# tuffy/libdvd-audio

Measured on AMD Instinct MI355X. Metric: decoded PCM Msamples/s (bit-exact) on 6ch/96k/24b MLP, higher is better.
Workload: dtype int32 (int64 accumulate)

## Files before the change

libdvd-audio_amd/csrc/mlp_decode.h:

```cpp
#pragma once
#include <hip/hip_runtime.h>
#if defined(__HIP_DEVICE_COMPILE__) && !defined(__gfx950__)
#error "mlp_decode.h is written for gfx950 (MI355X): hand-placed s_waitcnt encodings and gfx950 inline asm"
#endif
#include <stdint.h>
#include <type_traits>
#include "mlp_bounds.h"
#include "mlp_index.h"
#include "mlp_tables.h"

namespace mlp {

constexpr int DEC_THREADS = 128;
constexpr int DEC_WAVES = DEC_THREADS / 64;
constexpr int MAXCH = 8;
constexpr int MAXMAT = 6;
constexpr int RING_PLANES = 8;
constexpr int RING_DWORDS = RING_PLANES * 4;
constexpr int CHUNK_DWORDS = 16;
constexpr int OUT_ROWS = 4;
constexpr uint32_t YIELD_LONELY = 48;
#ifndef DVDA_HDR_GATE_TURNS
#define DVDA_HDR_GATE_TURNS 32
#endif
// ... 638 lines not shown
    Reader rx;
    rx.gsrc = rd.gsrc;
    rx.ring = &s_ring[wv][0][0][lane];
    rx.max_chunk = rd.max_chunk;
    rx.pos = 0;
    rx.fillpos = 0;
    rx.lo_valid = 0;
    SubPark P0;
    P0.flags = 0xFF;
    P0.block_size = 8;
    P0.min_ch = P0.max_ch = P0.max_mat_ch = P0.noise_shift = P0.seed = P0.matrix_len = P0.bypass_mask = P0.outch_pack = 0;
    P0.oshift_pack = P0.qss_pack = P0.nslots = P0.iir_any = P0.ss_end_bit = P0.rows_left = P0.blocks_in_frame = 0;
    P0.have_restart = false;
    P0.seg_iir = false;
    P0.gl = segi * 2u;
    P0.seg_lane = P0.gl;
    P0.chk = (DUO && active) ? DVDA_AT(a.seg_check, (size_t)segi * 2u, 2ull * a.caps.max_seg, BT_CHECK) : 0xFFFFFFFFu;
    P0.brec = P0.brec_end = P0.brec_base = nullptr;
    if (DUO && PARSE && active) {
        const uint4 pl = DVDA_AT(a.plan, segi, a.caps.max_seg + 1u, BT_PLAN);
        P0.brec = a.brec + brec_offset(pl.x, pl.y, 0u, seg_R);
        P0.brec_base = P0.brec;
        P0.brec_end = P0.brec + brec_capacity(seg_R);
        if (!DVDA_RANGE_OK(brec_offset(pl.x, pl.y, 0u, seg_R), brec_capacity(seg_R), a.caps.brec, BT_BREC)) {
            status |= ST_CAPACITY;
            active = false;
        }
    }

    uint64_t sp[NS][4];
    auto st_get = [&](int k, int j) -> int32_t {
        return (j & 1) ? (int32_t)(uint32_t)(sp[k][j >> 1] >> 32) : (int32_t)(uint32_t)sp[k][j >> 1];
    };
    auto st_set = [&](int k, int j, int32_t v) {
        if (j & 1)
            sp[k][j >> 1] = (sp[k][j >> 1] & 0xFFFFFFFFull) | ((uint64_t)(uint32_t)v << 32);
        else
            sp[k][j >> 1] = (sp[k][j >> 1] & 0xFFFFFFFF00000000ull) | (uint32_t)v;
    };
    constexpr bool CFU = !PARSE && !GENERAL && !DUO;
    constexpr int CFW = CFU ? 8 : 4;
    int32_t cf[NS][CFW];
    uint32_t pk[NS];
    int32_t sho[NS];
    uint32_t mreg[2][4];
    uint32_t mnoise[2] = {0, 0};
    constexpr bool MU = ILV && !PAIRED && !GENERAL && !PARSE && !DUO;
    int32_t mu[2][MU ? 8 : 1];
#pragma unroll
    for (int m = 0; m < 2; m++)
#pragma unroll
        for (int j = 0; j < (MU ? 8 : 1); j++)
            mu[m][j] = 0;
#pragma unroll
    for (int k = 0; k < NS; k++) {
#pragma unroll
        for (int j = 0; j < 4; j++)
            sp[k][j] = 0;
#pragma unroll
        for (int j = 0; j < CFW; j++)
            cf[k][j] = 0;
        pk[k] = hot_word(0u, 24u, 0u, 0u);
        s_cold[wv][k][lane] = (uint16_t)cold_word(0u, 0u, 0u, 0u);
        sho[k] = -(1 << 23);
    }
#pragma unroll
    for (int m = 0; m < 2; m++)
#pragma unroll
        for (int j = 0; j < 4; j++)
            mreg[m][j] = 0;
    if (GENERAL && resume_from_init) {
#pragma unroll
        for (int k = 0; k < NS; k++)
#pragma unroll
            for (int j = 0; j < 8; j++)
                st_set(k, j, a.init_fir[((size_t)sr.stream * 2 + sub) * 48 + k * 8 + j]);
    }
    uint32_t flags = 0xFF;
    uint32_t block_size = 8;
    uint32_t min_ch = 0, max_ch = 0, max_mat_ch = 0, noise_shift = 0, seed = 0;
    uint32_t matrix_len = 0, bypass_mask = 0, outch_pack = 0;
    uint32_t oshift_pack = 0, qss_pack = 0;
    uint32_t qss_A = 0, mmc_A = 0;
    uint32_t gate_turn = 0;
    auto no_restart_yet = [&]() -> uint32_t {
        if (GENERAL)
            return ST_ENVELOPE;
        const uint32_t first = a.streams[a.seg[segi].stream].first_seg;
        return segi != first ? ST_SEQ : ST_ENVELOPE;
    };
    constexpr bool HDR_GATE = !PAIRED && !GENERAL;
    const uint32_t gl_r = gl;
    uint32_t nslots = 0;
    bool have_restart = false;
    uint32_t iir_any = 0;
    bool seg_iir = false;

    uint64_t cur = sr.off;
    uint32_t ss_end_bit = 0;
    uint32_t rows_left = 0;
    bool in_frame = false;
    uint32_t frame_rows = 0;
    uint32_t blocks_in_frame = 0;
    uint32_t frames_done = 0;
    uint64_t row = row0;
    uint32_t rows_written = 0;
// ... 16 lines not shown
        sw(max_ch, P0.max_ch);
        sw(max_mat_ch, P0.max_mat_ch);
        sw(noise_shift, P0.noise_shift);
        sw(seed, P0.seed);
        sw(matrix_len, P0.matrix_len);
        sw(bypass_mask, P0.bypass_mask);
        sw(outch_pack, P0.outch_pack);
        sw(oshift_pack, P0.oshift_pack);
        sw(qss_pack, P0.qss_pack);
        sw(nslots, P0.nslots);
        sw(iir_any, P0.iir_any);
        sw(ss_end_bit, P0.ss_end_bit);
        sw(rows_left, P0.rows_left);
        sw(blocks_in_frame, P0.blocks_in_frame);
        sw(chk, P0.chk);
        sw(gl, P0.gl);
        sw(seg_lane, P0.seg_lane);
        swb(have_restart, P0.have_restart);
        swb(seg_iir, P0.seg_iir);
        swp(brec, P0.brec);
        swp(brec_end, P0.brec_end);
        swp(brec_base, P0.brec_base);
        dsub ^= 1u;
    };

    auto rematrix = [&](int32_t(&ch)[MAXCH], uint32_t bypass_bits) {
        const uint32_t shifted = (seed >> 7) & 0xFFFFu;
        const int32_t n0 = (int32_t)((uint32_t)(int32_t)(int8_t)(seed >> 15) << noise_shift);
        const int32_t n1 = (int32_t)((uint32_t)(int32_t)(int8_t)shifted << noise_shift);
        seed = (seed << 16) ^ shifted ^ (shifted << 5);
        auto one_matrix = [&](const uint32_t(&mc)[4], uint32_t nz, uint32_t m, bool on) {
            int64_t acc = (int64_t)n0 * (int64_t)lo16(nz) + (int64_t)n1 * (int64_t)hi16(nz);
#pragma unroll
            for (int c = 0; c < 6; c++)
                acc += (int64_t)ch[c] * (int64_t)((c & 1) ? hi16(mc[c >> 1]) : lo16(mc[c >> 1]));
            const uint32_t oc = nib(outch_pack, m);
            const int32_t nv = (int32_t)((uint32_t)mask_q((int32_t)(acc >> 14), nib(qss_A, oc)) +
                                         ((bypass_bits >> m) & 1u));
            uint32_t oce = on ? oc : 0xFFu;
            asm volatile("" : "+v"(oce));
            uint64_t hit[6];
#pragma unroll
            for (int c = 0; c < 6; c++) {
                hit[c] = __builtin_amdgcn_ballot_w64((uint32_t)c == oce);
                asm volatile("" : "+s"(hit[c]));
            }
#pragma unroll
            for (int c = 0; c < 6; c++) {
                int32_t keep = ch[c];
                asm("v_cndmask_b32_e64 %0, %0, %1, %2" : "+v"(keep) : "v"(nv), "s"(hit[c]));
                ch[c] = keep;
            }
        };
        auto one_matrix_u = [&](const int32_t(&c8)[MU ? 8 : 1], uint32_t m, bool on) {
            int64_t acc = (int64_t)n0 * (int64_t)c8[MU ? 6 : 0] + (int64_t)n1 * (int64_t)c8[MU ? 7 : 0];
#pragma unroll
            for (int c = 0; c < 6; c++)
                acc += (int64_t)ch[c] * (int64_t)c8[MU ? c : 0];
            const uint32_t oc = nib(outch_pack, m);
            const int32_t nv = (int32_t)((uint32_t)mask_q((int32_t)(acc >> 14), nib(qss_A, oc)) +
                                         ((bypass_bits >> m) & 1u));
            uint32_t oce = on ? oc : 0xFFu;
            asm volatile("" : "+v"(oce));
            uint64_t hit[6];
#pragma unroll
            for (int c = 0; c < 6; c++) {
                hit[c] = __builtin_amdgcn_ballot_w64((uint32_t)c == oce);
                asm volatile("" : "+s"(hit[c]));
            }
#pragma unroll
            for (int c = 0; c < 6; c++) {
                int32_t keep = ch[c];
                asm("v_cndmask_b32_e64 %0, %0, %1, %2" : "+v"(keep) : "v"(nv), "s"(hit[c]));
                ch[c] = keep;
            }
        };
        if constexpr (MU) {
            if (__any(matrix_len > 0))
                one_matrix_u(mu[0], 0, matrix_len > 0);
            if (__any(matrix_len > 1))
                one_matrix_u(mu[1], 1, matrix_len > 1);
        } else {
        if (__any(matrix_len > 0))
            one_matrix(mreg[0], mnoise[0], 0, matrix_len > 0);
        if (__any(matrix_len > 1))
            one_matrix(mreg[1], mnoise[1], 1, matrix_len > 1);
        }
        if (GENERAL && __builtin_expect(__any(matrix_len > 2), 0)) {
            for (uint32_t m = 2; m < matrix_len; m++) {
                DVDA_COV(9);
                uint32_t mc[4];
#pragma unroll
                for (int j = 0; j < 4; j++)
                    mc[j] = a.mat_ws[(size_t)(m * 5 + j) * a.total_lanes + gl_r];
                one_matrix(mc, a.mat_ws[(size_t)(m * 5 + 4) * a.total_lanes + gl_r], m, true);
            }
        }
        if (__any(oshift_pack != 0)) {
#pragma unroll
            for (int c = 0; c < MAXCH; c++)
                if ((uint32_t)c <= mmc_A)
                    ch[c] = (int32_t)((uint32_t)ch[c] << nib(oshift_pack, c));
        }
    };

#if defined(DVDA_EXP_STAMP)
    unsigned long long stamp_acc[8] = {0, 0, 0, 0, 0, 0, 0, 0};
    unsigned long long stamp_t = clock64();
    unsigned long long hstamp_acc[6] = {0, 0, 0, 0, 0, 0};
    unsigned long long hfills = 0, hcount = 0;
    unsigned long long hstamp_t = 0;
#endif
    for (;;) {
        DVDA_STAMP(5);
        bool hdr_parsed = false;
        bool hdr_now = active && (rows_left == 0 || (DUO && P0.rows_left == 0));
        if (HDR_GATE && __builtin_expect(__any(hdr_now), 0)) {
            const uint64_t m_need = __ballot(hdr_now), m_act = __ballot(active);
            const bool go = m_need == m_act || (uint32_t)__popcll(m_need) >= HDR_GATE_LANES ||
                            (gate_turn & (HDR_GATE_TURNS - 1u)) == 0u;
            hdr_now = hdr_now && go;
        }
        gate_turn++;
        if (__builtin_expect(hdr_now, 0)) {
#if defined(DVDA_EXP_STAMP)
            hstamp_t = clock64();
            rd.fill_cyc = rd.fill_n = 0;
            if constexpr (DUO)
                rx.fill_cyc = rx.fill_n = 0;
#endif
            while (active && !in_frame) {
                if (frames_done == sr.nframes) {
                    if (GENERAL && a.fir_ws) {
#pragma unroll
                        for (int k = 0; k < NS; k++)
#pragma unroll
                            for (int j = 0; j < 8; j++)
                                a.fir_ws[(size_t)(k * 8 + j) * a.total_lanes + seg_lane] = st_get(k, j);
                    }
                    if (GENERAL || PARSE)
                        a.seg_meta[seg_lane] = min_ch | (max_ch << 4) | (1u << 8) | (seg_iir ? 1u << 9 : 0u);
                    if (PARSE && brec) {
#pragma unroll
                        for (int kk = 0; kk < 6; kk++)
                            brec[BREC_SLOT * kk] = 0xFFFFFFFFu;
                    }
                    if constexpr (DUO && PARSE) {
                        a.seg_meta[P0.seg_lane] = P0.min_ch | (P0.max_ch << 4) | (1u << 8) | (P0.seg_iir ? 1u << 9 : 0u);
                        if (P0.brec) {
#pragma unroll
                            for (int kk = 0; kk < 6; kk++)
                                P0.brec[BREC_SLOT * kk] = 0xFFFFFFFFu;
                        }
                    }
                    bool go_on = false;
                    if (GENERAL) {
                        atomicOr(&a.seg_status[segi], status | ((status & ~ST_INFO) ? 0u : ST_GENERAL));
                        if (is_last_sub)
                            a.seg_rows[segi] = rows_written;
                        uint32_t nxt = segi + 1;
                        while (nxt < n_seg && a.seg[nxt].stream == sr.stream && (a.seg[nxt].flags & SEG_DEAD))
                            nxt++;
                        if (!(status & ~ST_INFO) && nxt < n_seg) {
                            const SegRec nr = DVDA_AT(a.seg, nxt, a.caps.max_seg, BT_SEG);
                            const uint32_t nst = DVDA_AT(a.seg_status, nxt, a.caps.max_seg, BT_STATUS);
                            if (nr.stream == sr.stream && !(nr.flags & ST_FATAL_INDEX) && nr.nframes &&
                                !(nst & ~ST_INFO)) {
                                go_on = true;
                                atomicAnd(&a.seg_status[nxt], ST_DEFERRED | ST_FATAL_INDEX | ST_TRUNCATED | ST_SYNC_CHANGE);
                                seg_lane += (nxt - segi) * 2u;
                                segi = nxt;
                                sr = nr;
                                cur = nr.off;
                                frames_done = 0;
                                drops_seen = 0;
                                rows_written = 0;
// ... 144 lines not shown
                        if (restart) {
                            flags = rd.read_resident(1) ? rd.read_resident(8) : 0xFFu;
                        } else if ((flags & 0x80u) && rd.read_resident(1)) {
                            flags = rd.read_resident(8);
                        }
                        if ((flags & 0x01u) && rd.read_resident(1)) {
                            block_size = rd.read_resident(9);
                            if (block_size < 8)
                                ok = false;
                        } else if (restart) {
                            block_size = 8;
                        }
                        if (ok && (flags & 0x02u) && rd.read_resident(1)) {
                            if (blocks_in_frame)
                                matrix_class_change = true;
                            matrix_len = rd.read_resident(4);
                            if (matrix_len > MAXMAT) {
                                ok = false;
                                err = ST_ENVELOPE;
                                matrix_len = 0;
                            }
                            bypass_mask = 0;
                            outch_pack = 0;
                            for (uint32_t m = 0; m < matrix_len && ok; m++) {
                                rd.ensure(HDR_MATRIX);
                                const uint32_t oc = rd.read_resident(4);
                                const uint32_t frac = rd.read_resident(4);
                                if (oc > max_mat_ch || frac > 14) {
                                    ok = false;
                                    break;
                                }
                                outch_pack |= oc << (4 * m);
                                bypass_mask |= rd.read_resident(1) << m;
                                uint32_t pair = 0, noise = 0;
                                for (uint32_t c = 0; c < 10; c++) {
                                    int32_t v = 0;
                                    if (c < max_mat_ch + 3 && rd.read_resident(1))
                                        v = (int32_t)((uint32_t)rd.read_signed_resident(frac + 2) << (14 - frac));
                                    if (c == max_mat_ch + 1)
                                        noise |= (uint32_t)v & 0xFFFFu;
                                    if (c == max_mat_ch + 2)
                                        noise |= (uint32_t)v << 16;
                                    const int32_t vc = c <= max_mat_ch ? v : 0;
                                    if (c & 1) {
                                        const uint32_t word = pair | ((uint32_t)vc << 16);
                                        if (c < 8) {
                                            a.mat_ws[(size_t)(m * 5 + (c >> 1)) * a.total_lanes + gl] = word;
#pragma unroll
                                            for (int mm = 0; mm < 2; mm++)
#pragma unroll
                                                for (int jj = 0; jj < 4; jj++)
                                                    if ((uint32_t)mm == m && (uint32_t)jj == (c >> 1) && mat_mine) {
                                                        mreg[mm][jj] = word;
                                                        if constexpr (MU) {
                                                            if (jj < 3) {
                                                                mu[mm][MU ? 2 * jj : 0] = lo16(word);
                                                                mu[mm][MU ? 2 * jj + 1 : 0] = hi16(word);
                                                            }
                                                        }
                                                    }
                                        }
                                    } else {
                                        pair = (uint32_t)vc & 0xFFFFu;
                                    }
                                }
                                a.mat_ws[(size_t)(m * 5 + 4) * a.total_lanes + gl] = noise;
                                if (m == 0 && mat_mine)
                                    mnoise[0] = noise;
                                if (m == 1 && mat_mine)
                                    mnoise[1] = noise;
                                if constexpr (MU) {
#pragma unroll
                                    for (int mm = 0; mm < 2; mm++)
                                        if ((uint32_t)mm == m && mat_mine) {
                                            mu[mm][MU ? 6 : 0] = lo16(noise);
                                            mu[mm][MU ? 7 : 0] = hi16(noise);
                                        }
                                }
                            }
                        } else if (restart) {
                            matrix_len = 0;
                            bypass_mask = 0;
                        }
                        if (ok && (flags & 0x04u) && rd.read_resident(1)) {
                            if (blocks_in_frame)
                                matrix_class_change = true;
                            for (uint32_t c = 0; c <= max_mat_ch; c++) {
                                const int32_t v = rd.read_signed_resident(4);
                                if (v < 0) {
                                    ok = false;
                                    err = ST_ENVELOPE;
                                }
                                oshift_pack = (oshift_pack & ~(0xFu << (4 * c))) | (((uint32_t)v & 0xFu) << (4 * c));
                            }
                        } else if (restart) {
                            oshift_pack = 0;
                        }
                        bool qss_changed = false;
                        if (ok && (flags & 0x08u) && rd.read_resident(1)) {
                            if (blocks_in_frame)
                                matrix_class_change = true;
                            for (uint32_t c = 0; c <= max_ch; c++)
                                qss_pack = (qss_pack & ~(0xFu << (4 * c))) | (rd.read_resident(4) << (4 * c));
                            qss_changed = true;
                        } else if (restart) {
                            qss_pack = 0;
                            qss_changed = true;
                        }
                        DVDA_HSTAMP(2);
                        for (uint32_t k = 0; k < nslots && ok; k++) {
                            rd.ensure(HDR_FIR);
                            const uint32_t c = min_ch + k;
                            const uint32_t kr = DUO ? c : k;
                            uint32_t pk_old = 0;
                            int32_t sho_old = 0;
                            uint32_t cf_old[4] = {0, 0, 0, 0};
#pragma unroll
                            for (int kk = 0; kk < NS; kk++)
                                if ((uint32_t)kk == kr) {
                                    pk_old = pk[kk];
                                    sho_old = sho[kk];
                                    if (PARSE) {
#pragma unroll
                                        for (int j = 0; j < 4; j++)
                                            cf_old[j] = !CFU ? (uint32_t)cf[kk][CFU ? 0 : j]
                                                             : (((uint32_t)cf[kk][CFU ? 2 * j : 0] & 0xFFFFu) |
                                                                ((uint32_t)cf[kk][CFU ? 2 * j + 1 : 0] << 16));
                                    }
                                }
                            uint32_t codebook = hot_cb(pk_old);
// ... 156 lines not shown
                                        const bool with_iir = new_iir && iir_order != 0;
                                        if (brec + 2 * BREC_STRIDE + (with_iir ? BREC_IIR_WORDS : 0) > brec_end) {
                                            seq_needed = true;
                                        } else {
                                            uint32_t *w = brec + BREC_SLOT * k;
                                            w[2] = shift | (q << 4) | (fir_order << 8) | (iir_order << 12) |
                                                   (new_iir ? 1u << 16 : 0u);
#pragma unroll
                                            for (int j = 0; j < 4; j++)
                                                w[3 + j] = new_fir ? ncf[j] : cf_old[j];
                                            w[7] = 0;
                                            chg_mask |= 1u << k;
                                            if (with_iir) {
                                                const int32_t *ws = a.iir_ws + (size_t)(k * 16) * a.total_lanes + gl;
                                                brec_end -= BREC_IIR_WORDS;
                                                uint32_t *x = brec_end;
                                                for (uint32_t j = 0; j < 4; j++)
                                                    x[j] = ((uint32_t)ws[(size_t)(2 * j) * a.total_lanes] & 0xFFFFu) |
                                                           ((uint32_t)ws[(size_t)(2 * j + 1) * a.total_lanes] << 16);
                                                for (uint32_t j = 0; j < 8; j++)
                                                    x[4 + j] = (uint32_t)ws[(size_t)(8 + j) * a.total_lanes];
                                                w[7] = (uint32_t)(x - brec_base);
                                            }
                                        }
                                    }
                                }
                            }
                        }
                    }
                }
                DVDA_HSTAMP(3);
                if (!have_restart && ok) {
                    ok = false;
                    err = no_restart_yet();
                }
                hdr_parsed = true;
                if (PARSE && iir_any)
                    seg_iir = true;
                if (PARSE && ok && chg_mask) {
#pragma unroll
                    for (int kk = 0; kk < 6; kk++) {
                        brec[BREC_SLOT * kk] = rows_done;
                        brec[BREC_SLOT * kk + 1] = (chg_mask >> kk) & 1u;
                    }
                    brec += BREC_STRIDE;
                }
                if (PARSE && ok && (seq_needed || (hdr_restart && blocks_in_frame))) {
                    status |= ST_SEQ;
                    active = false;
                }
                if (mat_mine) {
                    qss_A = qss_pack;
                    mmc_A = max_mat_ch;
                }
                const uint32_t cold_ml = matrix_len;
                if (matrix_class_change)
                    status |= ST_MIDFRAME;
                if (!ok) {
                    status |= err;
                    active = false;
                } else if (PARSE && !active) {
                } else if (!GENERAL && !PARSE && (iir_any != 0 || cold_ml > 2)) {
                    status |= ST_COLD;
                    active = false;
                } else if (!GENERAL && !PARSE && (status & ST_CHAINED)) {
                    active = false;
                    if (!(DUO && probe))
                        atomicAdd(&s_nchained[wv], 1u);
                    if (sr.prev != 0xFFFFFFFFu)
                        __hip_atomic_store(&DVDA_AT(a.yield_req, sr.prev, a.caps.max_seg, BT_YIELD), 1u, __ATOMIC_RELAXED, __HIP_MEMORY_SCOPE_AGENT);
                } else {
                    rows_left = block_size;
                    blocks_in_frame++;
                    if (!GENERAL && !PARSE && frames_done < 2 &&
                        __hip_atomic_load(&s_nchained[wv], __ATOMIC_RELAXED, __HIP_MEMORY_SCOPE_WORKGROUP) >= YIELD_LONELY) {
                        status |= ST_YIELD;
                        active = false;
                    }
                }
            }
                if constexpr (DUO) {
                    if (pass == 0u && me)
                        swap_sub();
                    if (!PARSE && pass == 0u && me && !active && first0 && !(status & ~ST_INFO)) {
                        probe = true;
                        active = true;
                    }
                    if (pass == 1u && probe)
                        active = false;
                }
            }
            if constexpr (DUO) {
                if (active && have_restart && P0.have_restart && (P0.min_ch != 0u || min_ch != P0.max_ch + 1u)) {
                    status |= PARSE ? ST_SEQ : ST_COLD;
                    active = false;
                }
            }
        }
        if (hdr_now) {
            DVDA_HSTAMP(4);
#if defined(DVDA_EXP_STAMP)
            hstamp_acc[5] += rd.fill_cyc + (DUO ? rx.fill_cyc : 0ull);
            hfills += rd.fill_n + (DUO ? rx.fill_n : 0ull);
            hcount++;
#endif
        }
        if (!__any(active))
            break;
        DVDA_STAMP(0);

        if (active) {
            if constexpr (DUO) {
                while (__builtin_expect(__any(rd.ahead() < 8 || rx.ahead() < 8), 0)) {
                    DVDA_COV(14);
                    uint4 q[1];
                    const int32_t n0 = rx.template fill_issue<1>(q);
                    rx.template fill_commit<1>(q, n0);
                    const int32_t n1 = rd.template fill_issue<1>(q);
                    rd.template fill_commit<1>(q, n1);
                }
            } else {
            if (rd.ahead() < 12)
                DVDA_COV(14);
            rd.ensure(12);
            }
        }
        DVDA_STAMP(7);
        constexpr int32_t FILL_TURN = 16;
        const bool pf = !WAVE_FILL && active && rd.room();
        const bool pfx = DUO && active && rx.room();
        int32_t fn = 0;
        uint4 p0, p1, p2, p3;
        asm volatile("" : "=v"(p0.x), "=v"(p0.y), "=v"(p0.z), "=v"(p0.w), "=v"(p1.x), "=v"(p1.y), "=v"(p1.z), "=v"(p1.w),
                          "=v"(p2.x), "=v"(p2.y), "=v"(p2.z), "=v"(p2.w), "=v"(p3.x), "=v"(p3.y), "=v"(p3.z), "=v"(p3.w));
        bool flush = false;
        const uint32_t frames_before = frames_done;
        uint64_t flush_row = 0;
        if constexpr (DUO) {
            if (pfx)
                p0 = rx.gsrc[rx.fill_src() >> 2];
            if (pf)
                p1 = rd.gsrc[rd.fill_src() >> 2];
        } else if constexpr (WAVE_FILL) {
            if (__any(active && rd.ahead() <= FILL_TURN)) {
                const int32_t r = (RD - rd.ahead()) >> 2;
                fn = active ? (r < 4 ? r : 4) : 0;
                const uint32_t end = rd.max_chunk + (uint32_t)CHUNK_DWORDS;
                const uint32_t last = end - 4u * (uint32_t)fn;
                const uint4 *src = rd.gsrc + ((rd.fillpos < last ? rd.fillpos : last) >> 2);
                if (fn > 0)
                    p0 = src[0];
                if (fn > 1)
                    p1 = src[1];
                if (fn > 2)
                    p2 = src[2];
                if (fn > 3)
                    p3 = src[3];
            }
        } else {
        if (pf) {
            const uint32_t c = rd.fillpos < rd.max_chunk ? rd.fillpos : rd.max_chunk;
            const uint4 *src = rd.gsrc + (c >> 2);
            p0 = src[0];
            p1 = src[1];
            p2 = src[2];
            p3 = src[3];
        }
        }
// ... 74 lines not shown
                    (void)wave_iir;
                } else {
                auto tap = [&](int j) -> int32_t {
                    if constexpr (CFU)
                        return cf[k][CFU ? j : 0];
                    else
                        return (j & 1) ? hi16((uint32_t)cf[k][CFU ? 0 : j >> 1]) : lo16((uint32_t)cf[k][CFU ? 0 : j >> 1]);
                };
                int64_t acc0 = (int64_t)tap(0) * (int64_t)st_get(k, 0);
                int64_t acc1 = (int64_t)tap(1) * (int64_t)st_get(k, 1);
                acc0 += (int64_t)tap(2) * (int64_t)st_get(k, 2);
                acc1 += (int64_t)tap(3) * (int64_t)st_get(k, 3);
                acc0 += (int64_t)tap(4) * (int64_t)st_get(k, 4);
                acc1 += (int64_t)tap(5) * (int64_t)st_get(k, 5);
                acc0 += (int64_t)tap(6) * (int64_t)st_get(k, 6);
                acc1 += (int64_t)tap(7) * (int64_t)st_get(k, 7);
                int64_t acc = acc0 + acc1;
                bool iir_on = false;
                if (__builtin_expect(wave_iir, 0)) {
                    iir_on = in && ((iir_any >> k) & 1u);
                    if (iir_on)
                        DVDA_COV(11);
                    if (iir_on)
                        acc += iir_mac(a.iir_ws + (size_t)(k * 16) * a.total_lanes + gl, a.total_lanes);
                }
                value = (int32_t)(((uint32_t)(acc >> ((hw >> 10) & 63u)) + resq) << q5);
                {
                    uint32_t vhi;
                    asm("" : "=v"(vhi));
                    const uint64_t vpair = (uint64_t)(uint32_t)value | ((uint64_t)vhi << 32);
                    asm("v_pk_mov_b32 %0, %1, %0 op_sel:[1,0]" : "+v"(sp[k][3]) : "v"(sp[k][2]));
                    asm("v_pk_mov_b32 %0, %1, %0 op_sel:[1,0]" : "+v"(sp[k][2]) : "v"(sp[k][1]));
                    asm("v_pk_mov_b32 %0, %1, %0 op_sel:[1,0]" : "+v"(sp[k][1]) : "v"(sp[k][0]));
                    asm("v_pk_mov_b32 %0, %1, %0 op_sel:[0,0]" : "+v"(sp[k][0]) : "v"(vpair));
                }
                if (__builtin_expect(wave_iir, 0)) {
                    if (iir_on) {
                        const int32_t ssum = (int32_t)(acc >> (((hw >> 10) & 63u) - hot_q(hw)));
                        iir_push(a.iir_ws + (size_t)(k * 16) * a.total_lanes + gl, a.total_lanes,
                                 (int32_t)((uint32_t)value - (uint32_t)ssum));
                    }
                }
                }
                val[k] = value;
                }
            }
            rd.pos = cpos;
            if (__builtin_expect((msb_or & 0x80u) != 0, 0)) {
                status |= ST_HUFFMAN;
                active = false;
            }
            DVDA_STAMP(2);
        };
        auto row_tail = [&](int32_t (&ch)[MAXCH]) {
            if (owner) {
                if (GENERAL) {
                    if (frame_rows >= (uint32_t)FB_ROWS) {
                        status |= ST_ENVELOPE;
                        active = false;
                    } else {
                        int32_t *fr = fbuf + (size_t)frame_rows * (MAXCH + 1);
#pragma unroll
                        for (int c = 0; c < MAXCH; c++)
                            fr[c] = ch[c];
                        fr[MAXCH] = (int32_t)bypass_bits;
                    }
                } else {
                    if constexpr (PARSE) {
#pragma unroll
                        for (int j = 0; j < OUT_ROWS - 1; j++) {
                            pq_s[j] = pq_s[j + 1];
                        }
                        pq_s[OUT_ROWS - 1] = (int32_t)((seed & 0x7FFFFFu) | (bypass_bits << 23));
                        const uint32_t shifted = (seed >> 7) & 0xFFFFu;
                        seed = (seed << 16) ^ shifted ^ (shifted << 5);
                    } else {
                        rematrix(ch, bypass_bits);
                    }
                    const uint32_t ph = rows_done & (OUT_ROWS - 1);
                    int32_t(*T)[OUT_ROWS][GENERAL ? 1 : 64] =
                        s_out[GENERAL ? 0 : wv];
                    if (ILV && ilv_direct) {
                        int32_t *Td = &T[0][0][GENERAL ? 0 : lane] + ph * (6 * 64);
#pragma unroll
                        for (int c = 0; c < 6; c++)
                            Td[c * 64] = ch[c];
                    } else {
#pragma unroll
                        for (int c = 0; c < TP; c++)
                            T[c][ph][GENERAL ? 0 : lane] = ch[c];
                    }
                    if (__builtin_expect(room == 0, 0)) {
                        if (row >= out_stride && row < row_limit) {
                            status |= ST_OVERFLOW;
                            active = false;
                        }
                    } else {
                        rows_written++;
                        if (ph == OUT_ROWS - 1) {
                            flush = true;
                            flush_row = row - (OUT_ROWS - 1);
                        }
                    }
                }
            }
            row++;
            rows_done++;
            if (GENERAL) {
                if (row > row_limit) {
                    status |= ST_TIMING;
                    active = false;
                }
            } else if (__builtin_expect(room == 0, 0)) {
                if (row > row_limit) {
                    status |= ST_TIMING;
                    active = false;
                }
            } else {
                room--;
            }
            frame_rows++;
            rows_left--;
            if constexpr (DUO) {
                P0.rows_left--;
                if (__builtin_expect(active && (rows_left == 0 || P0.rows_left == 0), 0)) {
                    bool last0 = false, last1 = false;
                    if (P0.rows_left == 0) {
                        last0 = rx.read(1) != 0;
                        if (rx.past(P0.ss_end_bit)) {
                            status |= ST_EOF;
                            active = false;
                        }
                        if (active && last0 && (P0.chk >> 2) == frames_done) {
                            status |= (P0.chk & 1u) ? ST_PARITY : ST_CRC;
                            active = false;
                        }
                    }
                    if (active && rows_left == 0) {
                        last1 = rd.read(1) != 0;
                        if (rd.past(ss_end_bit)) {
                            status |= ST_EOF;
                            active = false;
                        }
                        if (active && last1 && (chk >> 2) == frames_done) {
                            status |= (chk & 1u) ? ST_PARITY : ST_CRC;
                            active = false;
                        }
                    }
                    if (active && (last0 || last1) && (!(last0 && last1) || frame_rows != rpa)) {
                        status |= ST_TIMING;
                        active = false;
                    }
                    if (last0 && last1) {
                        if (PARSE && active) {
                            uint32_t *F = frec + (size_t)au_idx * FREC_WORDS;
                            if (!DVDA_RANGE_OK((size_t)(F - a.frec), FREC_WORDS, a.caps.frec, BT_FREC))
                                F = a.frec;
                            F[0] = noise_shift | (matrix_len << 8) | (max_mat_ch << 16);
                            F[1] = outch_pack;
                            F[2] = qss_pack;
                            F[3] = oshift_pack;
#pragma unroll
                            for (int m = 0; m < 2; m++) {
#pragma unroll
                                for (int j = 0; j < 4; j++)
                                    F[4 + m * 5 + j] = mreg[m][j];
                                F[4 + m * 5 + 4] = mnoise[m];
                            }
                            for (uint32_t m = 2; m < matrix_len; m++)
                                for (uint32_t j = 0; j < 5; j++)
                                    F[4 + m * 5 + j] = a.mat_ws[(size_t)(m * 5 + j) * a.total_lanes + gl];
                        }
// ... 55 lines not shown
                                    uint8_t *wb = reinterpret_cast<uint8_t *>(a.pcm + out_base) + orow * nch_out * nb;
                                    for (uint32_t c = 0; c < nch_out && c < 6u; c++) {
                                        int32_t v = 0;
#pragma unroll
                                        for (int cc = 0; cc < 6; cc++)
                                            if ((uint32_t)cc == c)
                                                v = ch[cc];
                                        const uint32_t u = wav_signed(v, a.wav_bits);
                                        for (uint32_t b = 0; b < nb; b++)
                                            wb[nib(wavepk, c) * nb + b] = (uint8_t)(u >> (8 * b));
                                    }
                                } else {
#pragma unroll
                                for (int c = 0; c < 6; c++)
                                    if ((uint32_t)c < nch_out)
                                        a.pcm[out_base + (a.interleaved ? orow * nch_out + nib(wavepk, c)
                                                                        : (uint64_t)nib(wavepk, c) * out_stride + orow)] = ch[c];
                                }
                            }
                            rows_written++;
                        }
                    }
                    in_frame = false;
                    frames_done++;
                } else if (rd.past(ss_end_bit)) {
                    status |= ST_EOF;
                    active = false;
                }
            }
        };
        int32_t ch[MAXCH];
        const bool in_row = active && (!HDR_GATE || (rows_left != 0 && (!DUO || P0.rows_left != 0)));
        if (in_row) {
            row_head_any();
            if (PAIRED) {
                const int slot0 = lane & ~1;
                int32_t(*X)[XCH ? 64 : 1] = s_xch[XCH ? wv : 0];
#pragma unroll
                for (int k = 0; k < NS; k++)
                    if ((uint32_t)k < nslots && min_ch + k < MAXCH)
                        X[min_ch + k][XCH ? slot0 : 0] = val[k];
                __builtin_amdgcn_fence(__ATOMIC_RELEASE, "wavefront");
                __builtin_amdgcn_wave_barrier();
                __builtin_amdgcn_fence(__ATOMIC_ACQUIRE, "wavefront");
#pragma unroll
                for (int c = 0; c < MAXCH; c++)
                    ch[c] = X[c][XCH ? slot0 : 0];
            } else {
#pragma unroll
                for (int c = 0; c < MAXCH; c++)
                    ch[c] = c < NS ? val[c < NS ? c : 0] : 0;
            }
            row_tail(ch);
        }
        if constexpr (GENERAL) {
            const int ended = frames_done != frames_before ? 1 : 0;
            const int other = __shfl_xor(ended, 1, 64);
            if (S == 2u && active && ended != other) {
                status |= ST_ENVELOPE;
                active = false;
            }
        }
        DVDA_STAMP(3);

#if defined(DVDA_EXP_STAMP)
        {
            asm volatile("s_waitcnt vmcnt(0)" ::: "memory");
            DVDA_STAMP(6);
        }
#endif
        __builtin_amdgcn_s_waitcnt(0x0F70);
        if constexpr (DUO) {
            if (pfx) {
                ring_store4<RD>(rx.slot(rx.fillpos), p0, (rx.fillpos & (RD - 1)) == 0);
                rx.filled();
            }
            if (pf) {
                ring_store4<RD>(rd.slot(rd.fillpos), p1, (rd.fillpos & (RD - 1)) == 0);
                rd.filled();
            }
        } else if constexpr (WAVE_FILL) {
            if (__any(fn > 0)) {
                const uint32_t f = rd.fillpos;
                if (fn > 0) {
                    ring_store4<RD>(rd.slot(f), p0, (f & (RD - 1)) == 0);
                    if (fn > 1) {
                        ring_store4<RD>(rd.slot(f + 4u), p1, ((f + 4u) & (RD - 1)) == 0);
                        if (fn > 2) {
                            ring_store4<RD>(rd.slot(f + 8u), p2, ((f + 8u) & (RD - 1)) == 0);
                            if (fn > 3)
                                ring_store4<RD>(rd.slot(f + 12u), p3, ((f + 12u) & (RD - 1)) == 0);
                        }
                    }
                    rd.fillpos = f + 4u * (uint32_t)fn;
                    if (rd.fillpos - rd.lo_valid > (uint32_t)RD)
                        rd.lo_valid = rd.fillpos - RD;
                }
            }
        } else {
        if (pf) {
            ring_store16(rd.slot(rd.fillpos), p0, p1, p2, p3, (rd.fillpos & (RING_DWORDS - 1)) == 0);
            rd.filled();
        }
        }
        bool coop_out = false;
        if constexpr (ILV && !GENERAL && !PARSE) {
            if (!WAVO && ilv_direct && a.wav_bits == 0u && a.coop_min_seg && n_seg >= a.coop_min_seg)
                coop_out = __ballot(flush) == ~0ull;
        }
        if (coop_out) {
            const uint64_t doff = out_base + flush_row * 6u;
            const bool off32 = !__any((doff >> 32) != 0);
            const uint32_t d_lo = (uint32_t)doff, d_hi = (uint32_t)(doff >> 32);
            const int32_t *const T0 = &s_out[GENERAL ? 0 : wv][0][0][0];
            const uint32_t l6 = ((uint32_t)lane * 43691u) >> 18;
            const uint32_t pc = (uint32_t)lane - l6 * 6u;
            const int32_t *const Tl6 = T0 + pc * (4 * 64) + l6;
            const bool l60 = lane < 60;
#pragma unroll
            for (uint32_t it7 = 0; it7 < 7u; it7++) {
                const uint32_t o = l6 + 10u * it7;
                const uint32_t b_lo = (uint32_t)__shfl((int)d_lo, (int)o, 64);
                uint64_t eo = b_lo;
                if (!off32)
                    eo |= (uint64_t)(uint32_t)__shfl((int)d_hi, (int)o, 64) << 32;
                if (l60 && (it7 < 6u || o < 64u)) {
                    int32_t *const od = a.pcm + eo + pc * 4u;
                    const int32_t *const Tp = Tl6 + 10u * it7;
                    DVDA_STORE_V4_COOP(od, Tp[0], Tp[64], Tp[128], Tp[192]);
                }
            }
        }
        if (!GENERAL && !PARSE && ILV && flush && !coop_out) {
            const int32_t *Tl = &s_out[GENERAL ? 0 : wv][0][0][GENERAL ? 0 : lane];
            int32_t *dst = a.pcm + out_base + flush_row * nch_out;
            constexpr bool WAV_ELSEWHERE = !PAIRED && !WAVO && !DUO;
            if (WAVO || (!WAV_ELSEWHERE && __builtin_expect(a.wav_bits != 0, 0))) {
                const uint32_t nb = a.wav_bits >> 3;
                uint32_t *wd = reinterpret_cast<uint32_t *>(a.pcm + out_base) + (flush_row * nch_out * nb >> 2);
                if (ilv_direct && a.wav_bits == 24u) {
                    uint32_t d[18];
#pragma unroll
                    for (int g = 0; g < 6; g++) {
                        const int32_t o[4] = {Tl[(4 * g) * 64], Tl[(4 * g + 1) * 64], Tl[(4 * g + 2) * 64], Tl[(4 * g + 3) * 64]};
                        uint32_t t[3];
                        wav_pack4(o, 24u, t);
                        d[3 * g] = t[0];
                        d[3 * g + 1] = t[1];
                        d[3 * g + 2] = t[2];
                    }
#pragma unroll
                    for (int v = 0; v < 4; v++)
                        DVDA_STORE_V4_AT(wd, 16 * v, (int)d[4 * v], (int)d[4 * v + 1], (int)d[4 * v + 2], (int)d[4 * v + 3]);
                    DVDA_STORE_V2_AT(wd, 64, d[16], d[17]);
                } else {
                    uint32_t fi = 0, fw = 0;
                    for (uint32_t v = 0; v < nch_out; v++) {
                        int32_t o[4];
#pragma unroll
                        for (int j = 0; j < 4; j++) {
                            o[j] = ilv_direct ? Tl[(4 * v + j) * 64] : Tl[(nib(wave_inv, fw) * OUT_ROWS + fi) * 64];
                            fw++;
                            if (fw == nch_out) {
                                fw = 0;
                                fi++;
                            }
                        }
                        uint32_t d[3];
                        wav_pack4(o, a.wav_bits, d);
                        wd[nb * v] = d[0];
                        wd[nb * v + 1] = d[1];
                        if (nb == 3u)
                            wd[nb * v + 2] = d[2];
                    }
                }
            } else if (__builtin_expect(ilv_direct, 1)) {
#pragma unroll
                for (int v = 0; v < (OUT_ROWS * 6) / 4; v++)
                    DVDA_STORE_V4_AT(dst, 16 * v, Tl[(4 * v) * 64], Tl[(4 * v + 1) * 64], Tl[(4 * v + 2) * 64],
                                     Tl[(4 * v + 3) * 64]);
            } else if (__all(nch_out == 2u && vec_ok)) {
                const int32_t *c0 = Tl + nib(wave_inv, 0) * (OUT_ROWS * 64), *c1 = Tl + nib(wave_inv, 1) * (OUT_ROWS * 64);
                DVDA_STORE_V4_AT(dst, 0, c0[0], c1[0], c0[64], c1[64]);
                DVDA_STORE_V4_AT(dst, 16, c0[128], c1[128], c0[192], c1[192]);
            } else {
                uint32_t fi = 0, fw = 0;
                for (uint32_t v = 0; v < (uint32_t)OUT_ROWS * 6u / 4u; v++) {
                    if (v * 4u < (uint32_t)OUT_ROWS * nch_out) {
                        int32_t o[4];
#pragma unroll
                        for (int j = 0; j < 4; j++) {
                            o[j] = Tl[(nib(wave_inv, fw) * OUT_ROWS + fi) * 64];
// ... 5 lines not shown
                        }
                        if (vec_ok) {
                            DVDA_STORE_V4(dst + 4 * v, o[0], o[1], o[2], o[3]);
                        } else {
#pragma unroll
                            for (int j = 0; j < 4; j++)
                                dst[4 * v + j] = o[j];
                            DVDA_COV(13);
                        }
                    }
                }
            }
        }
        bool coop_flush = false;
        if constexpr (PARSE && !GENERAL)
            coop_flush = __ballot(flush) == ~0ull;
        if (PARSE && flush) {
            int32_t(*T)[OUT_ROWS][GENERAL ? 1 : 64] = s_out[GENERAL ? 0 : wv];
            int32_t *dst = a.res + out_base + (flush_row >> 2) * 32u;
            if (!DVDA_RANGE_OK(out_base + (flush_row >> 2) * 32u, 32, a.caps.res, BT_RES))
                dst = a.res;
            if (!coop_flush) {
#pragma unroll
            for (int c = 0; c < TP; c++)
                DVDA_STORE_V4_AT(dst, 16 * c, T[c][0][GENERAL ? 0 : lane], T[c][1][GENERAL ? 0 : lane],
                                 T[c][2][GENERAL ? 0 : lane], T[c][3][GENERAL ? 0 : lane]);
            }
            DVDA_STORE_V4_AT(dst, 16 * 6, pq_s[0], pq_s[1], pq_s[2], pq_s[3]);
        }
        if constexpr (PARSE && !GENERAL) {
            if (coop_flush) {
                const int32_t *dsrc = a.res + out_base + (flush_row >> 2) * 32u;
                if (!flush || !DVDA_RANGE_OK(out_base + (flush_row >> 2) * 32u, 32, a.caps.res, BT_RES))
                    dsrc = a.res;
                const uint32_t d_lo = (uint32_t)(uintptr_t)dsrc, d_hi = (uint32_t)((uintptr_t)dsrc >> 32);
                const int32_t *const T0 = &s_out[wv][0][0][0];
                for (uint32_t it6 = 0; it6 < 6u; it6++) {
                    const uint32_t q = it6 * 64u + (uint32_t)lane;
                    const uint32_t o = (q * 43691u) >> 18;
                    const uint32_t pc = q - o * 6u;
                    const uint32_t b_lo = (uint32_t)__shfl((int)d_lo, (int)o, 64), b_hi = (uint32_t)__shfl((int)d_hi, (int)o, 64);
                    int32_t *const od = reinterpret_cast<int32_t *>(((uint64_t)b_hi << 32) | b_lo) + pc * 4u;
                    const int32_t *const Tp = T0 + pc * (OUT_ROWS * 64) + o;
                    DVDA_STORE_V4_PAD(od, Tp[0], Tp[64], Tp[128], Tp[192]);
                }
            }
        }
        if (!GENERAL && !PARSE && !ILV && flush) {
            int32_t(*T)[OUT_ROWS][GENERAL ? 1 : 64] = s_out[GENERAL ? 0 : wv];
#pragma unroll
            for (int c = 0; c < 6; c++) {
                if ((uint32_t)c < nch_out) {
                    const uint32_t wc = nib(wavepk, c);
                    int32_t *dst = a.pcm + out_base + (uint64_t)wc * out_stride + flush_row;
                    int32_t o[OUT_ROWS];
#pragma unroll
                    for (int i = 0; i < OUT_ROWS; i++)
                        o[i] = T[c][i][GENERAL ? 0 : lane];
                    if (vec_ok) {
#pragma unroll
                        for (int i = 0; i < OUT_ROWS; i += 4)
                            DVDA_STORE_V4(dst + i, o[i], o[i + 1], o[i + 2], o[i + 3]);
                    } else {
#pragma unroll
                        for (int i = 0; i < OUT_ROWS; i++)
                            dst[i] = o[i];
                        DVDA_COV(13);
                    }
                }
            }
        }
        DVDA_STAMP(4);
    }

#if defined(DVDA_EXP_STAMP)
    DVDA_STAMP(4);
    if (lane == 0 && a.dbg)
        for (int i = 0; i < 8; i++)
            atomicAdd(&a.dbg[i], stamp_acc[i]);
    if (lane == 0 && a.dbg)
        for (int i = 0; i < 6; i++)
            atomicAdd(&a.dbg[8 + i], hstamp_acc[i]);
    if (lane == 0 && a.dbg) {
        atomicAdd(&a.dbg[14], hfills);
        atomicAdd(&a.dbg[15], hcount);
    }
#endif
    if (!GENERAL && !PARSE && a.fir_ws && segi < n_seg && sub < S && frames_done == sr.nframes && sr.nframes) {
        if constexpr (DUO) {
#pragma unroll
            for (int k = 0; k < NS; k++) {
                const uint32_t s1 = (uint32_t)k >= min_ch ? 1u : 0u;
                const uint32_t kk = (uint32_t)k - (s1 ? min_ch : 0u);
                if ((uint32_t)k <= max_ch) {
#pragma unroll
                    for (int j = 0; j < 8; j++)
                        a.fir_ws[(size_t)(kk * 8 + j) * a.total_lanes + segi * 2u + s1] = st_get(k, j);
                }
            }
            a.seg_meta[segi * 2u] = P0.min_ch | (P0.max_ch << 4) | (1u << 8);
            a.seg_meta[segi * 2u + 1u] = min_ch | (max_ch << 4) | (1u << 8);
        } else {
#pragma unroll
        for (int k = 0; k < NS; k++)
#pragma unroll
            for (int j = 0; j < 8; j++)
                a.fir_ws[(size_t)(k * 8 + j) * a.total_lanes + gl] = st_get(k, j);
        a.seg_meta[gl] = min_ch | (max_ch << 4) | (1u << 8);
        }
    }
    uint32_t my_rows = 0;
    if (segi < n_seg && status) {
        const uint32_t old = atomicOr(&a.seg_status[segi], status);
        if (!GENERAL && !PARSE && (status & ST_CHAIN) && !(old & ST_CHAIN))
            my_rows = (sr.nframes - sr.ndrop) * rpa;
    }
    if (!GENERAL && !PARSE) {
        const uint64_t counted = __ballot(my_rows != 0);
        if (counted) {
            uint32_t lo = my_rows, hi = 0, mx = my_rows;
#pragma unroll
            for (int o = 32; o > 0; o >>= 1) {
                const uint32_t l2 = __shfl_xor(lo, o, 64), h2 = __shfl_xor(hi, o, 64), m2 = __shfl_xor(mx, o, 64);
                const uint32_t sum = lo + l2;
                hi += h2 + (sum < lo ? 1u : 0u);
                lo = sum;
                mx = mx > m2 ? mx : m2;
            }
            if (lane == 0) {
                DecodeSummary *const part = a.summary + 1 + (blockIdx.x % SUMMARY_PARTS);
                atomicAdd(&part->chain_segs, (uint32_t)__popcll(counted));
                atomicAdd(&part->chain_rows, ((unsigned long long)hi << 32) | lo);
                atomicMax(&part->chain_max_rows, mx);
            }
        }
    }
    if (segi < n_seg) {
        if (!GENERAL && !PARSE && owner && sub < S && mine)
            a.seg_rows[segi] = rows_written;
    }
}

constexpr uint32_t FIN_GROUP = 16;
__global__ __launch_bounds__(256) void k_finalize(const SegRec *__restrict__ seg,
                                                  const uint32_t *__restrict__ seg_fbase,
                                                  const uint32_t *__restrict__ seg_status,
                                                  const uint32_t *__restrict__ seg_rows,
                                                  StreamRec *__restrict__ streams, uint32_t n_streams,
                                                  DecodeSummary *__restrict__ summary,
                                                  uint32_t *__restrict__ seq_list, uint32_t collect, uint32_t last)
{
    const uint32_t t = blockIdx.x * blockDim.x + threadIdx.x;
    const uint32_t s = t / FIN_GROUP, j = t % FIN_GROUP;
    if (t == 0 && collect) {
        unsigned long long rows = 0;
        uint32_t segs = 0, mx = 0;
        for (uint32_t p = 1; p <= SUMMARY_PARTS; p++) {
            rows += summary[p].chain_rows;
            segs += summary[p].chain_segs;
            mx = summary[p].chain_max_rows > mx ? summary[p].chain_max_rows : mx;
            summary[p].chain_rows = 0;
            summary[p].chain_segs = 0;
            summary[p].chain_max_rows = 0;
        }
        summary->chain_rows += rows;
        summary->chain_segs += segs;
        summary->chain_max_rows = summary->chain_max_rows > mx ? summary->chain_max_rows : mx;
    }
    if (s >= n_streams)
        return;
    StreamRec r = streams[s];
    if (r.first_seg == 0xFFFFFFFFu) {
        r.status |= 1u << 0;
        r.frames = 0;
        r.rows = 0;
        r.n_seg = 0;
        r.consumed = 0;
    } else {
        uint64_t rows = 0;
        uint32_t st = r.status & ~(0x3FCu | ST_DEFERRED | ST_OVERFLOW | ST_GENERAL);
        uint32_t waits = 0;
        for (uint32_t i = r.first_seg + j; i < r.first_seg + r.n_seg; i += FIN_GROUP) {
            const uint32_t ss = seg_status[i];
            rows += seg_rows[i];
            st |= ss | (seg[i].flags & ~SEG_DEAD);
            if ((ss & ST_DEFERRED) && !(ss & ST_GENERAL) && !(ss & ~ST_INFO)) {
                waits = 1;
                if (last)
                    st |= ST_CAPACITY;
            }
        }
        uint32_t rlo = (uint32_t)rows, rhi = (uint32_t)(rows >> 32);
// ... 62 lines not shown
```

Measured before the change: 262,900.

## Fuse rematrix into row staging with precomputed output offsets and masks

For non-general decode paths, the per-row rematrix (two matrix MACs with ballot-based channel selection and cndmask writes) is replaced by direct MACs whose results are stored at precomputed shared-memory offsets, using quantisation masks precomputed per substream header. The dependence of matrix 1 on matrix 0's output channel is folded into a separate coefficient mk, so the ballots and the per-channel cndmask loop go away. Unpacked matrix coefficients are now rebuilt once per header wave instead of inside the parse loop. Row, overflow and timing bookkeeping are also reworked to be derived from rows_done and room. The added packing logic and changed bookkeeping add correctness risk on edge segments.

```diff
diff --git a/libdvd-audio_amd/csrc/mlp_decode.h b/libdvd-audio_amd/csrc/mlp_decode.h
--- a/libdvd-audio_amd/csrc/mlp_decode.h
+++ b/libdvd-audio_amd/csrc/mlp_decode.h
@@ -714,6 +714,14 @@
 #pragma unroll
         for (int j = 0; j < (MU ? 8 : 1); j++)
             mu[m][j] = 0;
+    constexpr bool PLACE = !GENERAL && !PARSE;
+    constexpr bool MPK = DUO;
+    uint32_t moff[2] = {0, 0};
+    uint32_t mqm[2] = {0xFFFFFFFFu, 0xFFFFFFFFu};
+    uint32_t mpk = 0;
+    int32_t mk = 0;
+    auto m_off = [&](int m) -> uint32_t { return MPK ? (mpk >> (11 * m)) & 0x7FFu : moff[m]; };
+    auto m_qm = [&](int m) -> uint32_t { return MPK ? 0xFFFFFFFFu << ((mpk >> (22 + 4 * m)) & 0xFu) : mqm[m]; };
 #pragma unroll
     for (int k = 0; k < NS; k++) {
 #pragma unroll
@@ -836,40 +844,10 @@
                 ch[c] = keep;
             }
         };
-        auto one_matrix_u = [&](const int32_t(&c8)[MU ? 8 : 1], uint32_t m, bool on) {
-            int64_t acc = (int64_t)n0 * (int64_t)c8[MU ? 6 : 0] + (int64_t)n1 * (int64_t)c8[MU ? 7 : 0];
-#pragma unroll
-            for (int c = 0; c < 6; c++)
-                acc += (int64_t)ch[c] * (int64_t)c8[MU ? c : 0];
-            const uint32_t oc = nib(outch_pack, m);
-            const int32_t nv = (int32_t)((uint32_t)mask_q((int32_t)(acc >> 14), nib(qss_A, oc)) +
-                                         ((bypass_bits >> m) & 1u));
-            uint32_t oce = on ? oc : 0xFFu;
-            asm volatile("" : "+v"(oce));
-            uint64_t hit[6];
-#pragma unroll
-            for (int c = 0; c < 6; c++) {
-                hit[c] = __builtin_amdgcn_ballot_w64((uint32_t)c == oce);
-                asm volatile("" : "+s"(hit[c]));
-            }
-#pragma unroll
-            for (int c = 0; c < 6; c++) {
-                int32_t keep = ch[c];
-                asm("v_cndmask_b32_e64 %0, %0, %1, %2" : "+v"(keep) : "v"(nv), "s"(hit[c]));
-                ch[c] = keep;
-            }
-        };
-        if constexpr (MU) {
-            if (__any(matrix_len > 0))
-                one_matrix_u(mu[0], 0, matrix_len > 0);
-            if (__any(matrix_len > 1))
-                one_matrix_u(mu[1], 1, matrix_len > 1);
-        } else {
         if (__any(matrix_len > 0))
             one_matrix(mreg[0], mnoise[0], 0, matrix_len > 0);
         if (__any(matrix_len > 1))
             one_matrix(mreg[1], mnoise[1], 1, matrix_len > 1);
-        }
         if (GENERAL && __builtin_expect(__any(matrix_len > 2), 0)) {
             for (uint32_t m = 2; m < matrix_len; m++) {
                 DVDA_COV(9);
@@ -906,6 +884,18 @@
             hdr_now = hdr_now && go;
         }
         gate_turn++;
+        const bool hdr_wave = MU && __any(hdr_now);
+        if constexpr (MU) {
+            if (hdr_wave) {
+#pragma unroll
+                for (int m = 0; m < 2; m++) {
+#pragma unroll
+                    for (int j = 0; j < 3; j++)
+                        mreg[m][j] = ((uint32_t)mu[m][MU ? 2 * j : 0] & 0xFFFFu) | ((uint32_t)mu[m][MU ? 2 * j + 1 : 0] << 16);
+                    mnoise[m] = ((uint32_t)mu[m][MU ? 6 : 0] & 0xFFFFu) | ((uint32_t)mu[m][MU ? 7 : 0] << 16);
+                }
+            }
+        }
         if (__builtin_expect(hdr_now, 0)) {
 #if defined(DVDA_EXP_STAMP)
             hstamp_t = clock64();
@@ -1156,12 +1146,6 @@
                                                 for (int jj = 0; jj < 4; jj++)
                                                     if ((uint32_t)mm == m && (uint32_t)jj == (c >> 1) && mat_mine) {
                                                         mreg[mm][jj] = word;
-                                                        if constexpr (MU) {
-                                                            if (jj < 3) {
-                                                                mu[mm][MU ? 2 * jj : 0] = lo16(word);
-                                                                mu[mm][MU ? 2 * jj + 1 : 0] = hi16(word);
-                                                            }
-                                                        }
                                                     }
                                         }
                                     } else {
@@ -1173,13 +1157,20 @@
                                     mnoise[0] = noise;
                                 if (m == 1 && mat_mine)
                                     mnoise[1] = noise;
-                                if constexpr (MU) {
-#pragma unroll
-                                    for (int mm = 0; mm < 2; mm++)
-                                        if ((uint32_t)mm == m && mat_mine) {
-                                            mu[mm][MU ? 6 : 0] = lo16(noise);
-                                            mu[mm][MU ? 7 : 0] = hi16(noise);
-                                        }
+                            }
+                            if constexpr (PLACE) {
+                                if (mat_mine) {
+                                    mk = 0;
+                                    if (matrix_len > 1) {
+                                        const uint32_t oc0 = outch_pack & 0xFu;
+#pragma unroll
+                                        for (int jj = 0; jj < 3; jj++)
+                                            if ((uint32_t)jj == (oc0 >> 1)) {
+                                                const uint32_t word = mreg[1][jj];
+                                                mk = (oc0 & 1u) ? hi16(word) : lo16(word);
+                                                mreg[1][jj] = word & ((oc0 & 1u) ? 0x0000FFFFu : 0xFFFF0000u);
+                                            }
+                                    }
                                 }
                             }
                         } else if (restart) {
@@ -1442,6 +1433,20 @@
                 if (mat_mine) {
                     qss_A = qss_pack;
                     mmc_A = max_mat_ch;
+                    if constexpr (PLACE) {
+                        mpk = 0;
+#pragma unroll
+                        for (int m = 0; m < 2; m++) {
+                            const uint32_t oc = nib(outch_pack, m);
+                            const uint32_t off = oc * ((ILV && ilv_direct) ? 64u : (uint32_t)(OUT_ROWS * 64));
+                            if constexpr (MPK) {
+                                mpk |= (off << (11 * m)) | (nib(qss_pack, oc) << (22 + 4 * m));
+                            } else {
+                                moff[m] = off;
+                                mqm[m] = 0xFFFFFFFFu << nib(qss_pack, oc);
+                            }
+                        }
+                    }
                 }
                 const uint32_t cold_ml = matrix_len;
                 if (matrix_class_change)
@@ -1487,6 +1492,20 @@
                 }
             }
         }
+        if constexpr (MU) {
+            if (hdr_wave) {
+#pragma unroll
+                for (int m = 0; m < 2; m++) {
+#pragma unroll
+                    for (int j = 0; j < 3; j++) {
+                        mu[m][MU ? 2 * j : 0] = lo16(mreg[m][j]);
+                        mu[m][MU ? 2 * j + 1 : 0] = hi16(mreg[m][j]);
+                    }
+                    mu[m][MU ? 6 : 0] = lo16(mnoise[m]);
+                    mu[m][MU ? 7 : 0] = hi16(mnoise[m]);
+                }
+            }
+        }
         if (hdr_now) {
             DVDA_HSTAMP(4);
 #if defined(DVDA_EXP_STAMP)
@@ -1504,6 +1523,7 @@
                 while (__builtin_expect(__any(rd.ahead() < 8 || rx.ahead() < 8), 0)) {
                     DVDA_COV(14);
                     uint4 q[1];
+                    asm volatile("" : "=v"(q[0].x), "=v"(q[0].y), "=v"(q[0].z), "=v"(q[0].w));
                     const int32_t n0 = rx.template fill_issue<1>(q);
                     rx.template fill_commit<1>(q, n0);
                     const int32_t n1 = rd.template fill_issue<1>(q);
@@ -1684,6 +1704,7 @@
             }
             DVDA_STAMP(2);
         };
+        const bool no_room = PLACE && room == 0;
         auto row_tail = [&](int32_t (&ch)[MAXCH]) {
             if (owner) {
                 if (GENERAL) {
@@ -1697,8 +1718,84 @@
                             fr[c] = ch[c];
                         fr[MAXCH] = (int32_t)bypass_bits;
                     }
+                } else if constexpr (PLACE) {
+                    const uint32_t shifted = (seed >> 7) & 0xFFFFu;
+                    const int32_t n0 = (int32_t)((uint32_t)(int32_t)(int8_t)(seed >> 15) << noise_shift);
+                    const int32_t n1 = (int32_t)((uint32_t)(int32_t)(int8_t)shifted << noise_shift);
+                    seed = (seed << 16) ^ shifted ^ (shifted << 5);
+                    const uint32_t ph = rows_done & (OUT_ROWS - 1);
+                    const bool on0 = matrix_len > 0, on1 = matrix_len > 1;
+                    const uint64_t any0 = __ballot(on0), any1 = __ballot(on1);
+                    auto stage_row = [&](auto with_shifts, auto frame_major) {
+                        constexpr bool OSH = decltype(with_shifts)::value;
+                        constexpr bool FM = decltype(frame_major)::value;
+                        int32_t *const Tb = &s_out[wv][0][0][lane] + ph * (FM ? 6u * 64u : 64u);
+                        auto out_c = [&](int c) -> int32_t {
+                            if constexpr (OSH)
+                                return (uint32_t)c <= mmc_A ? (int32_t)((uint32_t)ch[c] << nib(oshift_pack, c)) : ch[c];
+                            else
+                                return ch[c];
+                        };
+                        auto out_m = [&](uint32_t m, int32_t nv) -> int32_t {
+                            if constexpr (OSH) {
+                                const uint32_t oc = nib(outch_pack, m);
+                                return oc <= mmc_A ? (int32_t)((uint32_t)nv << nib(oshift_pack, oc)) : nv;
+                            } else {
+                                return nv;
+                            }
+                        };
+                        auto mac = [&](int m) -> int64_t {
+                            int64_t acc;
+                            if constexpr (MU) {
+                                acc = (int64_t)n0 * (int64_t)mu[m][MU ? 6 : 0] + (int64_t)n1 * (int64_t)mu[m][MU ? 7 : 0];
+#pragma unroll
+                                for (int c = 0; c < 6; c++)
+                                    acc += (int64_t)ch[c] * (int64_t)mu[m][MU ? c : 0];
+                            } else {
+                                acc = (int64_t)n0 * (int64_t)lo16(mnoise[m]) + (int64_t)n1 * (int64_t)hi16(mnoise[m]);
+#pragma unroll
+                                for (int c = 0; c < 6; c++)
+                                    acc += (int64_t)ch[c] * (int64_t)((c & 1) ? hi16(mreg[m][c >> 1]) : lo16(mreg[m][c >> 1]));
+                            }
+                            return acc;
+                        };
+                        if constexpr (FM) {
+#pragma unroll
+                            for (int c = 0; c < 6; c++)
+                                Tb[c * 64] = out_c(c);
+                        } else {
+#pragma unroll
+                            for (int c = 0; c < TP; c++)
+                                Tb[c * (OUT_ROWS * 64)] = out_c(c);
+                        }
+                        if (any0) {
+                            const int32_t nv0 = (int32_t)(((uint32_t)(int32_t)(mac(0) >> 14) & m_qm(0)) + (bypass_bits & 1u));
+                            if (on0)
+                                Tb[m_off(0)] = out_m(0, nv0);
+                            if (any1) {
+                                const int64_t acc = mac(1) + (int64_t)nv0 * (int64_t)mk;
+                                const int32_t nv1 = (int32_t)(((uint32_t)(int32_t)(acc >> 14) & m_qm(1)) + ((bypass_bits >> 1) & 1u));
+                                if (on1)
+                                    Tb[m_off(1)] = out_m(1, nv1);
+                            }
+                        }
+                    };
+                    const bool osh = __any(oshift_pack != 0);
+                    if (ILV && ilv_direct) {
+                        if constexpr (ILV) {
+                            if (__builtin_expect(osh, 0))
+                                stage_row(std::true_type{}, std::true_type{});
+                            else
+                                stage_row(std::false_type{}, std::true_type{});
+                        }
+                    } else {
+                        if (__builtin_expect(osh, 0))
+                            stage_row(std::true_type{}, std::false_type{});
+                        else
+                            stage_row(std::false_type{}, std::false_type{});
+                    }
                 } else {
-                    if constexpr (PARSE) {
+                    {
 #pragma unroll
                         for (int j = 0; j < OUT_ROWS - 1; j++) {
                             pq_s[j] = pq_s[j + 1];
@@ -1706,8 +1803,6 @@
                         pq_s[OUT_ROWS - 1] = (int32_t)((seed & 0x7FFFFFu) | (bypass_bits << 23));
                         const uint32_t shifted = (seed >> 7) & 0xFFFFu;
                         seed = (seed << 16) ^ shifted ^ (shifted << 5);
-                    } else {
-                        rematrix(ch, bypass_bits);
                     }
                     const uint32_t ph = rows_done & (OUT_ROWS - 1);
                     int32_t(*T)[OUT_ROWS][GENERAL ? 1 : 64] =
@@ -1736,20 +1831,41 @@
                     }
                 }
             }
-            row++;
-            rows_done++;
-            if (GENERAL) {
-                if (row > row_limit) {
-                    status |= ST_TIMING;
-                    active = false;
-                }
-            } else if (__builtin_expect(room == 0, 0)) {
-                if (row > row_limit) {
-                    status |= ST_TIMING;
-                    active = false;
-                }
+            if constexpr (PLACE) {
+                if (__builtin_expect(__any(no_room), 0)) {
+                    if (no_room) {
+                        const uint64_t row_now = row0 + rows_done;
+                        if (owner && row_now >= out_stride && row_now < row_limit) {
+                            status |= ST_OVERFLOW;
+                            active = false;
+                        }
+                        if (row_now + 1u > row_limit) {
+                            status |= ST_TIMING;
+                            active = false;
+                        }
+                    } else {
+                        room--;
+                    }
+                } else {
+                    room--;
+                }
+                rows_done++;
             } else {
-                room--;
+                row++;
+                rows_done++;
+                if (GENERAL) {
+                    if (row > row_limit) {
+                        status |= ST_TIMING;
+                        active = false;
+                    }
+                } else if (__builtin_expect(room == 0, 0)) {
+                    if (row > row_limit) {
+                        status |= ST_TIMING;
+                        active = false;
+                    }
+                } else {
+                    room--;
+                }
             }
             frame_rows++;
             rows_left--;
@@ -1911,6 +2027,8 @@
                     ch[c] = c < NS ? val[c < NS ? c : 0] : 0;
             }
             row_tail(ch);
+            if constexpr (PLACE)
+                flush = owner && !no_room && (rows_done & (OUT_ROWS - 1)) == 0;
         }
         if constexpr (GENERAL) {
             const int ended = frames_done != frames_before ? 1 : 0;
@@ -1962,13 +2080,14 @@
             rd.filled();
         }
         }
+        auto out_row = [&]() -> uint64_t { return PLACE ? row0 + rows_done - (uint64_t)OUT_ROWS : flush_row; };
         bool coop_out = false;
         if constexpr (ILV && !GENERAL && !PARSE) {
             if (!WAVO && ilv_direct && a.wav_bits == 0u && a.coop_min_seg && n_seg >= a.coop_min_seg)
                 coop_out = __ballot(flush) == ~0ull;
         }
         if (coop_out) {
-            const uint64_t doff = out_base + flush_row * 6u;
+            const uint64_t doff = out_base + out_row() * 6u;
             const bool off32 = !__any((doff >> 32) != 0);
             const uint32_t d_lo = (uint32_t)doff, d_hi = (uint32_t)(doff >> 32);
             const int32_t *const T0 = &s_out[GENERAL ? 0 : wv][0][0][0];
@@ -1992,11 +2111,11 @@
         }
         if (!GENERAL && !PARSE && ILV && flush && !coop_out) {
             const int32_t *Tl = &s_out[GENERAL ? 0 : wv][0][0][GENERAL ? 0 : lane];
-            int32_t *dst = a.pcm + out_base + flush_row * nch_out;
+            int32_t *dst = a.pcm + out_base + out_row() * nch_out;
             constexpr bool WAV_ELSEWHERE = !PAIRED && !WAVO && !DUO;
             if (WAVO || (!WAV_ELSEWHERE && __builtin_expect(a.wav_bits != 0, 0))) {
                 const uint32_t nb = a.wav_bits >> 3;
-                uint32_t *wd = reinterpret_cast<uint32_t *>(a.pcm + out_base) + (flush_row * nch_out * nb >> 2);
+                uint32_t *wd = reinterpret_cast<uint32_t *>(a.pcm + out_base) + (out_row() * nch_out * nb >> 2);
                 if (ilv_direct && a.wav_bits == 24u) {
                     uint32_t d[18];
 #pragma unroll
@@ -2108,7 +2227,7 @@
             for (int c = 0; c < 6; c++) {
                 if ((uint32_t)c < nch_out) {
                     const uint32_t wc = nib(wavepk, c);
-                    int32_t *dst = a.pcm + out_base + (uint64_t)wc * out_stride + flush_row;
+                    int32_t *dst = a.pcm + out_base + (uint64_t)wc * out_stride + out_row();
                     int32_t o[OUT_ROWS];
 #pragma unroll
                     for (int i = 0; i < OUT_ROWS; i++)
@@ -2192,8 +2311,13 @@
         }
     }
     if (segi < n_seg) {
-        if (!GENERAL && !PARSE && owner && sub < S && mine)
-            a.seg_rows[segi] = rows_written;
+        if (!GENERAL && !PARSE && owner && sub < S && mine) {
+            uint32_t room0 = 0;
+            const uint64_t edge = out_stride < row_limit ? out_stride : row_limit;
+            if (edge > row0)
+                room0 = edge - row0 > 0xFFFFFFFFull ? 0xFFFFFFFFu : (uint32_t)(edge - row0);
+            a.seg_rows[segi] = room0 - room;
+        }
     }
 }
 
```

Measured after the change: 267,200, median of 6. About the same (+1.6%).
